# ubc-vision/StableKeypoints

Measured on AMD Instinct MI355X. Metric: images/sec for token-optimization step (SD1.5, 512^2, K=10 kpts), higher is better.
Workload: dtype f32 (fp32 MFMA / VALU throughout; flash attention of the >= 1024-key self-attention layers: 3xbf16 operand split, fp32 accumulate, error <= the fp32 kernel's)

## Files before the change

### include/skp.h

```cpp
#ifndef SKP_H
#define SKP_H

#include <stdint.h>

#ifdef __cplusplus
extern "C" {
#endif

#define SKP_MAX_LAYERS 8
#define SKP_MAX_SUBJECTS 4

#define SKP_E_BADARG (-1)
#define SKP_E_RANGE  (-2)
#define SKP_E_LDS    (-3)

int skp_abi_version(void);

int skp_tune_set(const char* key, int value);
int skp_tune_get(const char* key);

int skp_gemm_nt_f32(const float* A, const float* B, float* C, int M, int N, int K, int Z0, int Z1,
                    int64_t sa0, int64_t sa1, int64_t sam, int64_t sak,
                    int64_t sb0, int64_t sb1, int64_t sbn, int64_t sbk,
                    int64_t sc0, int64_t sc1, int64_t scm, float alpha, void* stream);
// ... 22 lines not shown
int64_t skp_attn_map_bwd_col_workspace(const int* s , int L, int B, int H, int T, int R, int K);
int skp_attn_map_bwd_col_f32(const float* const* S , float* const* dS , const int* s , int L,
                             int B, int H, int T, int R, const int64_t* sel, const float* G, int K, const float* lse,
                             void* workspace, int ldt, void* stream);

int64_t skp_attn_map_bwd_sparse_workspace(const int* s , int L, int B, int H, int T, int R, int K);
int skp_attn_map_bwd_sparse_f32(const float* const* S , float* const* dS , const int* s ,
                                int L, int B, int H, int T, int R, const int64_t* sel, const float* G, int K,
                                const float* lse, void* workspace, int ldt, void* stream);

int skp_unwarp_accumulate_f32(const float* M, const float* theta_inv, int n, int K, int R, int S, float* tot, float* num,
                              int finish, void* stream);

int skp_group_norm_coef_f32(const float* x, const float* off, const float* gamma, const float* beta, float* mean, float* rstd,
                            float* coef, const float* bs, int nblk, int pix, float* workspace, int N, int C, int G, int HW,
                            float eps, void* stream);
int skp_conv3x3_f4_gn_ok(int B, int Cin, int Cout, int H, int W);
int skp_conv3x3_f4_gn_f32(const void* x, const void* U, const void* bias, const void* residual, void* y, float* stats,
                          const float* coef, int B, int Cin, int Cout, int H, int W, void* stream);

int skp_conv3x3_f4r_ok(int B, int Cin, int Cout, int H, int W);
int skp_conv3x3_f4r_filter_f32(const void* w, void* R, int Cout, int Cin, int flip_transpose, void* stream);
int64_t skp_conv3x3_f4r_workspace(int B, int Cin, int Cout, int H, int W);
int skp_conv3x3_f4r_f32(const void* x, const void* R, const void* bias, const void* residual, void* y, void* workspace,
                        int B, int Cin, int Cout, int H, int W, void* stream);

int skp_cross_attn_fwd_f32(const float* q, const float* k, const float* v, float* out, float* lse,
                           int B, int Bk, int H, int N, int T, int d, float scale, void* stream);
int64_t skp_cross_attn_bwd_workspace(int B, int H, int N, int T, int d);
int skp_cross_attn_bwd_f32(const float* q, const float* k, const float* v, const float* out,
                           const float* dout, const float* lse, float* dq, float* dk, float* dv,
                           float* workspace, int B, int Bk, int H, int N, int T, int d, float scale,
                           void* stream);

int skp_attn_map_bwd_ex_f32(const float* const* S , float* const* dS , const int* s ,
                            int L, int B, int H, int T, int R, const float* dM, const float* lse,
                            float* workspace, float* dot_io, int ldt, int64_t m_bstride, int mode, void* stream);

int64_t skp_flash_attn_bwd_workspace(int B, int Bk, int H, int N, int Nk, int d);
int skp_flash_attn_fwd_f32(const float* q, const float* k, const float* v, float* out, float* lse,
                           int B, int Bk, int H, int N, int Nk, int d, float scale, void* stream);
int skp_flash_attn_bwd_f32(const float* q, const float* k, const float* v, const float* out, const float* dout,
                           const float* lse, float* dq, float* dk, float* dv, float* workspace,
                           int B, int Bk, int H, int N, int Nk, int d, float scale, void* stream);
int skp_flash_attn_bwd_ld_f32(const float* q, const float* k, const float* v, const float* out, const float* dout,
                              const float* lse, float* dq, float* dk, float* dv, float* workspace,
                              int B, int Bk, int H, int N, int Nk, int d, float scale, int ldg, void* stream);

int skp_flash_attn_fwd_split_ok(int B, int Bk, int H, int N, int Nk, int d);
int64_t skp_flash_attn_fwd_split_workspace(int B, int Bk, int H, int N, int Nk, int d);
int skp_flash_attn_fwd_split_f32(const float* q, const float* k, const float* v, float* out, float* lse, void* workspace,
                                 int B, int Bk, int H, int N, int Nk, int d, float scale, void* stream);
int skp_flash_attn_bwd_split_ok(int B, int Bk, int H, int N, int Nk, int d);
int64_t skp_flash_attn_bwd_split_workspace(int B, int Bk, int H, int N, int Nk, int d);
int skp_flash_attn_bwd_split_f32(const float* q, const float* k, const float* v, const float* out, const float* dout,
                                 const float* lse, float* dq, float* dk, float* dv, void* workspace, int B, int Bk, int H, int N,
                                 int Nk, int d, float scale, void* stream);
int skp_flash_attn_bwd_split_ld_f32(const float* q, const float* k, const float* v, const float* out, const float* dout,
                                    const float* lse, float* dq, float* dk, float* dv, void* workspace, int B, int Bk, int H,
                                    int N, int Nk, int d, float scale, int ldg, void* stream);

int skp_self_attn_fwd_f32(const float* q, const float* k, const float* v, float* out, float* lse,
                          int B, int H, int N, int d, float scale, void* stream);
int skp_self_attn_bwd_f32(const float* q, const float* k, const float* v, const float* out, const float* dout,
                          const float* lse, float* dq, float* dk, float* dv, float* workspace,
                          int B, int H, int N, int d, float scale, void* stream);
// ... 100 lines not shown
```

### stablekeypoints_amd/_native.py

```python
from __future__ import annotations

import ctypes as C
import os

import torch

_HERE = os.path.dirname(os.path.abspath(__file__))
LIB_PATH = os.environ.get("SKP_LIB_PATH") or os.path.join(_HERE, "csrc", "libskp_hip.so")
ABI_VERSION = 41

_vp, _i, _f, _i64 = C.c_void_p, C.c_int, C.c_float, C.c_int64

SIGNATURES = {
    "skp_abi_version": [],
    "skp_tune_set": [C.c_char_p, _i],
    "skp_tune_get": [C.c_char_p],
    "skp_group_norm_onepass_ok": [_i, _i, _i, _i],
    "skp_gemm_nt_f32": [_vp, _vp, _vp, _i, _i, _i, _i, _i,
                        _i64, _i64, _i64, _i64, _i64, _i64, _i64, _i64, _i64, _i64, _i64, _f, _vp],
    "skp_qk_logits_f32": [_vp, _vp, _vp, _i, _i, _i, _i, _i, _i, _f, _vp],
    "skp_attn_map_fwd_f32": [C.POINTER(_vp), C.POINTER(_i), _i, _i, _i, _i, _i, _vp, _vp, _vp],
    "skp_attn_map_fwd_ex_f32": [C.POINTER(_vp), C.POINTER(_i), _i, _i, _i, _i, _i, _vp, _vp, _vp, _i, _i64, _i, _vp],
    "skp_attn_map_bwd_ex_f32": [C.POINTER(_vp), C.POINTER(_vp), C.POINTER(_i), _i, _i, _i, _i, _i, _vp, _vp, _vp, _vp,
                                _i, _i64, _i, _vp],
    "skp_attn_map_bwd_workspace": [C.POINTER(_i), _i, _i, _i, _i, _i],
    "skp_attn_map_bwd_f32": [C.POINTER(_vp), C.POINTER(_vp), C.POINTER(_i), _i, _i, _i, _i, _i, _vp, _vp, _vp, _vp],
    "skp_group_norm_coef_f32": [_vp, _vp, _vp, _vp, _vp, _vp, _vp, _vp, _i, _i, _vp, _i, _i, _i, _i, _f, _vp],
    "skp_conv3x3_f4_gn_ok": [_i, _i, _i, _i, _i],
    "skp_conv3x3_f4_gn_f32": [_vp, _vp, _vp, _vp, _vp, _vp, _vp, _i, _i, _i, _i, _i, _vp],
    "skp_unwarp_accumulate_f32": [_vp, _vp, _i, _i, _i, _i, _vp, _vp, _i, _vp],
    "skp_attn_map_fwd_wide_f32": [C.POINTER(_vp), C.POINTER(_i), _i, _i, _i, _i, _i, _vp, _vp, _vp, _i, _i, _vp],
    "skp_attn_map_fwd_wide_ok": [C.POINTER(_i), _i, _i, _i],
    "skp_attn_map_bwd_col_ok": [C.POINTER(_i), _i, _i, _i, _i, _i],
    "skp_attn_map_bwd_col_workspace": [C.POINTER(_i), _i, _i, _i, _i, _i, _i],
    "skp_attn_map_bwd_col_f32": [C.POINTER(_vp), C.POINTER(_vp), C.POINTER(_i), _i, _i, _i, _i, _i, _vp, _vp, _i, _vp, _vp,
                                 _i, _vp],
    "skp_attn_map_bwd_sparse_workspace": [C.POINTER(_i), _i, _i, _i, _i, _i, _i],
    "skp_attn_map_bwd_sparse_f32": [C.POINTER(_vp), C.POINTER(_vp), C.POINTER(_i), _i, _i, _i, _i, _i, _vp, _vp, _i, _vp, _vp,
                                    _i, _vp],
    "skp_token_stats_f32": [_vp, _i, _i, _i, _f, _f, _vp, _vp, _vp, _vp],
    "skp_select_tokens": [_vp, _vp, _i, _i, _i, _i, _vp, _vp, _vp],
    "skp_select_tokens_batched": [_vp, _vp, _i, _i, _i, _i, _i, _vp, _vp, _vp],
    "skp_losses_fwd_f32": [_vp, _vp, _vp, _i, _i, _i, _vp, _i, _f, C.POINTER(_f), _vp, _vp, _vp, _vp, _vp],
    "skp_losses_fwd_dev_f32": [_vp, _vp, _vp, _i, _i, _i, _vp, _i, _f, _vp, _vp, _vp, _vp, _vp, _vp],
    "skp_rows_axpy_f32": [_vp, _vp, _i, _i64, _vp, _vp, _vp, _vp, _vp],
    "skp_cross_attn_fwd_f32": [_vp, _vp, _vp, _vp, _vp, _i, _i, _i, _i, _i, _i, _f, _vp],
    "skp_cross_attn_bwd_workspace": [_i, _i, _i, _i, _i],
    "skp_cross_attn_bwd_f32": [_vp, _vp, _vp, _vp, _vp, _vp, _vp, _vp, _vp, _vp, _i, _i, _i, _i, _i, _i, _f, _vp],
    "skp_group_norm_fwd_f32": [_vp, _vp, _vp, _vp, _vp, _vp, _vp, _vp, _i, _i, _i, _i, _f, _i, _vp],
    "skp_group_norm_bwd_f32": [_vp, _vp, _vp, _vp, _vp, _vp, _vp, _vp, _vp, _i, _i, _i, _i, _f, _i, _vp],
    "skp_group_norm_bwd_add_f32": [_vp, _vp, _vp, _vp, _vp, _vp, _vp, _vp, _vp, _vp, _i, _i, _i, _i, _f, _i, _vp],
    "skp_add_bias_residual_f32": [_vp, _vp, _vp, _vp, _i, _i, _i, _vp],
    "skp_add_layer_norm_ok": [_i],
    "skp_add_layer_norm_fwd_f32": [_vp, _vp, _vp, _vp, _vp, _vp, _vp, _i64, _i, _f, _vp],
    "skp_add_layer_norm_bwd_f32": [_vp, _vp, _vp, _vp, _vp, _vp, _i64, _i, _vp],
    "skp_conv3x3_filter_f32": [_vp, _vp, _i, _i, _i, _vp],
    "skp_conv3x3_workspace": [_i, _i, _i, _i, _i, _i],
    "skp_conv3x3_f32": [_vp, _vp, _vp, _vp, _vp, _vp, _i, _i, _i, _i, _i, _i, _vp],
    "skp_conv3x3_f4_filter_f32": [_vp, _vp, _i, _i, _i, _vp],
    "skp_conv3x3_f4_workspace": [_i, _i, _i, _i, _i],
    "skp_conv3x3_f4_f32": [_vp, _vp, _vp, _vp, _vp, _vp, _i, _i, _i, _i, _i, _vp],
    "skp_flash_attn_fwd_split_ok": [_i, _i, _i, _i, _i, _i],
    "skp_flash_attn_fwd_split_workspace": [_i, _i, _i, _i, _i, _i],
    "skp_flash_attn_fwd_split_f32": [_vp, _vp, _vp, _vp, _vp, _vp, _i, _i, _i, _i, _i, _i, C.c_float, _vp],
    "skp_flash_attn_bwd_split_ok": [_i, _i, _i, _i, _i, _i],
    "skp_flash_attn_bwd_split_workspace": [_i, _i, _i, _i, _i, _i],
    "skp_flash_attn_bwd_split_f32": [_vp, _vp, _vp, _vp, _vp, _vp, _vp, _vp, _vp, _vp, _i, _i, _i, _i, _i, _i, _f, _vp],
    "skp_flash_attn_bwd_split_ld_f32": [_vp, _vp, _vp, _vp, _vp, _vp, _vp, _vp, _vp, _vp, _i, _i, _i, _i, _i, _i, _f, _i, _vp],
    "skp_conv3x3_f4r_ok": [_i, _i, _i, _i, _i],
    "skp_conv3x3_f4r_filter_f32": [_vp, _vp, _i, _i, _i, _vp],
    "skp_conv3x3_f4r_workspace": [_i, _i, _i, _i, _i],
    "skp_conv3x3_f4r_f32": [_vp, _vp, _vp, _vp, _vp, _vp, _i, _i, _i, _i, _i, _vp],
    "skp_conv3x3_s2_filter_f32": [_vp, _vp, _i, _i, _vp],
    "skp_conv3x3_s2_f32": [_vp, _vp, _vp, _vp, _i, _i, _i, _i, _i, _i, _vp],
    "skp_conv3x3_s2_workspace": [_i, _i, _i, _i, _i],
    "skp_conv3x3_s2_ws_f32": [_vp, _vp, _vp, _vp, _vp, _i, _i, _i, _i, _i, _i, _vp],
    "skp_conv3x3_s2w_ok": [_i, _i, _i, _i, _i, _i],
    "skp_conv3x3_s2w_filter_f32": [_vp, _vp, _i, _i, _i, _vp],
    "skp_conv3x3_s2w_f32": [_vp, _vp, _vp, _vp, _i, _i, _i, _i, _i, _i, _vp],
    "skp_conv3x3_s2w_stats_f32": [_vp, _vp, _vp, _vp, _vp, _i, _i, _i, _i, _i, _i, _vp],
    "skp_conv3x3_small_f32": [_vp, _vp, _vp, _vp, _i, _i, _i, _i, _i, _vp],
# ... 102 lines not shown
```

### stablekeypoints_amd/csrc/skp_common.h

```cpp
#pragma once
#include <hip/hip_runtime.h>
#include <stdint.h>
#include "../../include/skp.h"

#define SKP_WAVE 64
#define SKP_LOG2E 1.4426950408889634f

typedef float f32x16 __attribute__((ext_vector_type(16)));
typedef float f32x4 __attribute__((ext_vector_type(4)));
typedef float f32x2 __attribute__((ext_vector_type(2)));

enum { SKP_TUNE_WINO_SPLIT = 0, SKP_TUNE_WINO_RAW_MAX_TILES, SKP_TUNE_MAP_BANDS, SKP_TUNE_FA2_TWO_KERNEL_BWD, SKP_TUNE_GN_FOLD_MAX_COUT, SKP_TUNE_CROSS_ATTN_TS,
       SKP_TUNE_CONV_S2W, SKP_TUNE_CONV_UP2, SKP_TUNE_COUNT };
int skp_tune(int key);

static inline int skp_launch_status() {
    hipError_t e = hipGetLastError();
    return e == hipSuccess ? 0 : (int)e;
}

__device__ __forceinline__ void skp_cubic_taps(int dst, float ratio, int n, int idx[4], float w[4]) {
    const float A = -0.75f;
    const float src = ratio * ((float)dst + 0.5f) - 0.5f;
    const float fl = floorf(src);
    const float t = src - fl;
    const int i0 = (int)fl;
    float x = t + 1.0f;
    w[0] = ((A * x - 5.0f * A) * x + 8.0f * A) * x - 4.0f * A;
    x = t;
    w[1] = ((A + 2.0f) * x - (A + 3.0f)) * x * x + 1.0f;
    x = 1.0f - t;
    w[2] = ((A + 2.0f) * x - (A + 3.0f)) * x * x + 1.0f;
    x = 2.0f - t;
    w[3] = ((A * x - 5.0f * A) * x + 8.0f * A) * x - 4.0f * A;
#pragma unroll
    for (int i = 0; i < 4; ++i) {
        int v = i0 - 1 + i;
        idx[i] = v < 0 ? 0 : (v > n - 1 ? n - 1 : v);
    }
}

__device__ __forceinline__ float skp_wave_sum(float v) {
#pragma unroll
    for (int o = 32; o > 0; o >>= 1) v += __shfl_xor(v, o, 64);
    return v;
}
// ... 34 lines not shown
```

### stablekeypoints_amd/csrc/skp_cross_attn.hip

```cpp
#include "skp_attn_tiles.h"

#define SKP_CA_KSPLIT_MAX 16

int skp_gemm_nt_splitk(const float* A, const float* B, float* C, float* partial, int64_t c_elems, int ksplit,
                       int M, int N, int K, int Z0, int Z1,
                       int64_t sa0, int64_t sa1, int64_t sam, int64_t sak,
                       int64_t sb0, int64_t sb1, int64_t sbn, int64_t sbk,
                       int64_t sc0, int64_t sc1, int64_t scm, float alpha, void* stream);

static int ca_ksplit(int N) { int k = N / 256; return k < 1 ? 1 : (k > SKP_CA_KSPLIT_MAX ? SKP_CA_KSPLIT_MAX : k); }

template <int D8, int TT>
__global__ __launch_bounds__(256) void skp_cross_attn_fwd_kernel(const float* __restrict__ q, const float* __restrict__ k,
                                                                 const float* __restrict__ v, float* __restrict__ out,
                                                                 float* __restrict__ lse, int Bk, int H, int N, int T,
                                                                 float scale) {
    using S = CAShape<D8, TT>;
    extern __shared__ __attribute__((aligned(16))) float smem[];
    const int tid = threadIdx.x, wave = tid >> 6, lane = tid & 63, i = lane & 31, hi = lane >> 5;
    const int b = blockIdx.z, h = blockIdx.y, C = H * S::D;
    const int n0 = blockIdx.x * 128 + wave * 32, n = n0 + i;
    const bool nv = n < N;
    const float* qrow = q + ((size_t)b * N + (nv ? n : N - 1)) * C + h * S::D;
    const float sl2 = scale * SKP_LOG2E;
// ... 271 lines not shown
    const float lse2 = lse[((size_t)b * H + h) * N + (nv ? n : N - 1)] * SKP_LOG2E;
#pragma unroll
    for (int r = 0; r < 16; ++r) p[0][r] = (t0 + ca_tok(0, r, hi) < T) ? __builtin_amdgcn_exp2f(p[0][r] - lse2) : 0.f;
    ca_stage_wave<D8>(reg, v + kvoff, t0, T, C, lane);
    {
        f32x4 dov[D8];
#pragma unroll
        for (int j = 0; j < D8; ++j) {
            dov[j] = *(const f32x4*)(dout + rowoff + 8 * j + 4 * hi);
            const f32x4 ov = *(const f32x4*)(out + rowoff + 8 * j + 4 * hi);
            dsum += dov[j][0] * ov[0] + dov[j][1] * ov[1] + dov[j][2] * ov[2] + dov[j][3] * ov[3];
        }
        dsum += __shfl_xor(dsum, 32, 64);
#pragma unroll
        for (int r = 0; r < 16; ++r) dp[0][r] = 0.f;
        ca_swapped_product<D8, 1>(reg, dov, dp, i, hi);
    }
    const size_t stb = ((size_t)b * H + h) * TP * N;
#pragma unroll
    for (int r = 0; r < 16; ++r) {
        dp[0][r] = p[0][r] * (dp[0][r] - dsum);
        if (nv) {
            const size_t o = stb + (size_t)(t0 + ca_tok(0, r, hi)) * N + n;
            Pst[o] = p[0][r];
            dSst[o] = dp[0][r];
        }
    }
    ca_stage_wave<D8>(reg, k + kvoff, t0, T, C, lane);
    f32x16 o[S::CT];
    ca_reg_product<D8, 1>(reg, dp, o, i, hi);
    ca_merge_store<D8, NW>(smem, reg, o, dq, scale, b, h, H, N, n0, wave, lane);
}

static bool ca_use_ts(int B, int H, int N, int T, int d) {
    if (skp_tune(SKP_TUNE_CROSS_ATTN_TS) == 1) return false;
    const int tt = (T + 31) / 32;
    if (tt < 2 || !(d == 80 || d == 160)) return false;
    return (long)((N + 127) / 128) * H * B * 4 < 1024;
}

static int ca_check(int B, int Bk, int H, int N, int T, int d) {
    if (B <= 0 || H <= 0 || N <= 0 || T <= 0 || d <= 0 || (Bk != 1 && Bk != B)) return SKP_E_BADARG;
    if (T > 128 || B > 65535 || H > 65535) return SKP_E_RANGE;
    if (d != 8 && d != 16 && d != 32 && d != 40 && d != 64 && d != 80 && d != 160) return SKP_E_RANGE;
    return 0;
}

#define SKP_CA_DISPATCH(KERNEL, ...)                                                                     \
    {                                                                                                    \
        const int tt = (T + 31) / 32;                                                                    \
        const int tsel = tt <= 1 ? 1 : (tt <= 3 ? 3 : 4);                                                \
        dim3 grid((N + 127) / 128, H, B), block(256);                                                    \
        hipStream_t st = (hipStream_t)stream;                                                            \
        int launched = 0;                                                                                \
        SKP_CA_CASE(KERNEL, 1, 1, __VA_ARGS__) SKP_CA_CASE(KERNEL, 1, 3, __VA_ARGS__) SKP_CA_CASE(KERNEL, 1, 4, __VA_ARGS__)     \
        SKP_CA_CASE(KERNEL, 2, 1, __VA_ARGS__) SKP_CA_CASE(KERNEL, 2, 3, __VA_ARGS__) SKP_CA_CASE(KERNEL, 2, 4, __VA_ARGS__)     \
        SKP_CA_CASE(KERNEL, 4, 1, __VA_ARGS__) SKP_CA_CASE(KERNEL, 4, 3, __VA_ARGS__) SKP_CA_CASE(KERNEL, 4, 4, __VA_ARGS__)     \
        SKP_CA_CASE(KERNEL, 5, 1, __VA_ARGS__) SKP_CA_CASE(KERNEL, 5, 3, __VA_ARGS__) SKP_CA_CASE(KERNEL, 5, 4, __VA_ARGS__)     \
        SKP_CA_CASE(KERNEL, 8, 1, __VA_ARGS__) SKP_CA_CASE(KERNEL, 8, 3, __VA_ARGS__) SKP_CA_CASE(KERNEL, 8, 4, __VA_ARGS__)     \
        SKP_CA_CASE(KERNEL, 10, 1, __VA_ARGS__) SKP_CA_CASE(KERNEL, 10, 3, __VA_ARGS__) SKP_CA_CASE(KERNEL, 10, 4, __VA_ARGS__)  \
        SKP_CA_CASE(KERNEL, 20, 1, __VA_ARGS__) SKP_CA_CASE(KERNEL, 20, 3, __VA_ARGS__) SKP_CA_CASE(KERNEL, 20, 4, __VA_ARGS__)  \
        if (!launched) return SKP_E_RANGE;                                                               \
    }

#define SKP_CA_CASE(KERNEL, D8V, TTV, ...)                                                               \
    if (!launched && d == D8V * 8 && tsel == TTV) {                                                      \
// ... 7 lines not shown
        launched = 1;                                                                                    \
    }

#define SKP_CA_TS_CASE(KERNEL, D8V, NWV, ...)                                                            \
    if (!launched && d == D8V * 8 && nw == NWV) {                                                        \
        const size_t lds = ((size_t)NWV * CATS<D8V>::REG + 2 * NWV * 32) * sizeof(float);                \
        if (lds > 64 * 1024) {                                                                           \
            hipError_t e = hipFuncSetAttribute((const void*)KERNEL<D8V, NWV>,                            \
                                               hipFuncAttributeMaxDynamicSharedMemorySize, (int)lds);    \
            if (e != hipSuccess) return (int)e;                                                          \
        }                                                                                                \
        hipLaunchKernelGGL((KERNEL<D8V, NWV>), dim3((N + 31) / 32, H, B), dim3(64 * NWV), lds, (hipStream_t)stream, __VA_ARGS__); \
        launched = 1;                                                                                    \
    }
#define SKP_CA_TS_DISPATCH(KERNEL, ...)                                                                  \
    {                                                                                                    \
        const int nw = (T + 31) / 32 <= 3 ? ((T + 31) / 32 <= 2 ? 2 : 3) : 4;                            \
        int launched = 0;                                                                                \
        SKP_CA_TS_CASE(KERNEL, 10, 2, __VA_ARGS__) SKP_CA_TS_CASE(KERNEL, 10, 3, __VA_ARGS__) SKP_CA_TS_CASE(KERNEL, 10, 4, __VA_ARGS__) \
        SKP_CA_TS_CASE(KERNEL, 20, 2, __VA_ARGS__) SKP_CA_TS_CASE(KERNEL, 20, 3, __VA_ARGS__) SKP_CA_TS_CASE(KERNEL, 20, 4, __VA_ARGS__) \
        if (!launched) return SKP_E_RANGE;                                                               \
    }

extern "C" int skp_cross_attn_tp(int T) {
    const int tt = (T + 31) / 32;
    return (tt <= 1 ? 1 : (tt <= 3 ? 3 : 4)) * 32;
}

extern "C" int64_t skp_cross_attn_bwd_workspace(int B, int H, int N, int T, int d) {
    if (B <= 0 || H <= 0 || N <= 0 || T <= 0 || T > 128 || d <= 0) return SKP_E_BADARG;
    return (2 * (int64_t)B * H * skp_cross_attn_tp(T) * N + (int64_t)ca_ksplit(N) * B * T * H * d) * (int64_t)sizeof(float);
}

extern "C" int skp_cross_attn_fwd_f32(const float* q, const float* k, const float* v, float* out, float* lse,
                                      int B, int Bk, int H, int N, int T, int d, float scale, void* stream) {
    if (!q || !k || !v || !out || !lse) return SKP_E_BADARG;
    int rc = ca_check(B, Bk, H, N, T, d);
    if (rc) return rc;
    if (ca_use_ts(B, H, N, T, d)) {
        SKP_CA_TS_DISPATCH(skp_cross_attn_fwd_ts_kernel, q, k, v, out, lse, Bk, H, N, T, scale)
        return skp_launch_status();
    }
    SKP_CA_DISPATCH(skp_cross_attn_fwd_kernel, q, k, v, out, lse, Bk, H, N, T, scale)
    return skp_launch_status();
}

extern "C" int skp_cross_attn_bwd_f32(const float* q, const float* k, const float* v, const float* out,
                                      const float* dout, const float* lse, float* dq, float* dk, float* dv,
                                      float* workspace, int B, int Bk, int H, int N, int T, int d, float scale,
                                      void* stream) {
    if (!q || !k || !v || !out || !dout || !lse || !dq || !dk || !dv || !workspace) return SKP_E_BADARG;
    int rc = ca_check(B, Bk, H, N, T, d);
    if (rc) return rc;
    const int TP = skp_cross_attn_tp(T);
    float* Pst = workspace;
    float* dSst = workspace + (size_t)B * H * TP * N;
    if (ca_use_ts(B, H, N, T, d)) {
        SKP_CA_TS_DISPATCH(skp_cross_attn_bwd_ts_kernel, q, k, v, out, dout, lse, dq, Pst, dSst, Bk, H, N, T, TP, scale)
    } else {
        SKP_CA_DISPATCH(skp_cross_attn_bwd_kernel, q, k, v, out, dout, lse, dq, Pst, dSst, Bk, H, N, T, scale)
    }
    rc = skp_launch_status();
    if (rc) return rc;
    const int64_t C = (int64_t)H * d;
    float* part = dSst + (size_t)B * H * TP * N;
    const int ksp = ca_ksplit(N);
// ... 8 lines not shown
```

### stablekeypoints_amd/csrc/skp_select_loss.hip

```cpp
#include "skp_common.h"
#include <string.h>

__device__ __forceinline__ bool skp_better(float v, int i, float bv, int bi) {
    return (v > bv) || (v == bv && i < bi);
}

struct StatsArgs { int T, R, S; float sigma, eps; };

__global__ __launch_bounds__(256) void skp_token_stats_kernel(const float* __restrict__ M, StatsArgs a,
                                                              int32_t* __restrict__ argmax_out,
                                                              float* __restrict__ kl_out, float* __restrict__ ent_out) {
    __shared__ float red_v[4];
    __shared__ int red_i[4];
    __shared__ float red[4];
    __shared__ float s_cy[SKP_MAX_SUBJECTS], s_cx[SKP_MAX_SUBJECTS];
    const int t = blockIdx.x, tid = threadIdx.x, R = a.R, RR = R * R;
    const float* m = M + (size_t)t * RR;
    const float rad = 0.05f * (float)R;
    const float rad2 = rad * rad;
    float maxval0 = 0.f;
    for (int j = 0; j < a.S; ++j) {
        float bv = -INFINITY; int bi = 0x7fffffff;
        for (int p = tid; p < RR; p += 256) {
            const int row = p / R, col = p - row * R;
// ... 338 lines not shown
                                  const int32_t* argmax, int num_subjects, float sigma, const float* theta_inv,
                                  float* partial, float* g_sharp, float* g_eq_a, float* g_eq_b, void* stream) {
    return losses_run(M, Mt, sel, K, T, R, argmax, num_subjects, sigma, theta_inv, nullptr, partial, g_sharp, g_eq_a, g_eq_b, stream);
}

extern "C" int skp_losses_fwd_dev_f32(const float* M, const float* Mt, const int64_t* sel, int K, int T, int R,
                                      const int32_t* argmax, int num_subjects, float sigma, const float* theta_inv_dev,
                                      float* partial, float* g_sharp, float* g_eq_a, float* g_eq_b, void* stream) {
    if (!theta_inv_dev) return SKP_E_BADARG;
    return losses_run(M, Mt, sel, K, T, R, argmax, num_subjects, sigma, nullptr, theta_inv_dev, partial, g_sharp, g_eq_a, g_eq_b, stream);
}

__global__ __launch_bounds__(256) void skp_rows_axpy_kernel(float* __restrict__ dst, const int64_t* __restrict__ sel,
                                                            int64_t n, const float* __restrict__ x,
                                                            const float* __restrict__ a, const float* __restrict__ y,
                                                            const float* __restrict__ b) {
    const int k = blockIdx.y;
    const int64_t i = (int64_t)blockIdx.x * 256 + threadIdx.x;
    if (i >= n) return;
    float v = a[0] * x[(size_t)k * n + i];
    if (y) v += b[0] * y[(size_t)k * n + i];
    dst[(size_t)sel[k] * n + i] += v;
}

extern "C" int skp_rows_axpy_f32(float* dst, const int64_t* sel, int K, int64_t n, const float* x, const float* a,
                                 const float* y, const float* b, void* stream) {
    if (!dst || !sel || !x || !a || K <= 0 || n <= 0 || (y && !b)) return SKP_E_BADARG;
    if (K > 65535) return SKP_E_RANGE;
    hipLaunchKernelGGL(skp_rows_axpy_kernel, dim3((unsigned)((n + 255) / 256), K), dim3(256), 0, (hipStream_t)stream,
                       dst, sel, n, x, a, y, b);
    return skp_launch_status();
}

extern "C" int skp_abi_version(void) { return 41; }

static int g_tune[SKP_TUNE_COUNT] = {0};
static const char* const g_tune_names[SKP_TUNE_COUNT] = {"wino_split", "wino_raw_max_tiles", "map_bands", "fa2_two_kernel_bwd", "gn_fold_max_cout", "cross_attn_ts", "conv_s2w", "conv_up2"};
int skp_tune(int key) { return (key >= 0 && key < SKP_TUNE_COUNT) ? g_tune[key] : 0; }
extern "C" int skp_tune_set(const char* key, int value) {
    if (!key || value < 0) return SKP_E_BADARG;
    for (int i = 0; i < SKP_TUNE_COUNT; ++i)
        if (!strcmp(key, g_tune_names[i])) { g_tune[i] = value; return 0; }
    return SKP_E_RANGE;
}
extern "C" int skp_tune_get(const char* key) {
    if (!key) return SKP_E_BADARG;
    for (int i = 0; i < SKP_TUNE_COUNT; ++i)
        if (!strcmp(key, g_tune_names[i])) return g_tune[i];
    return SKP_E_RANGE;
}
```

### stablekeypoints_amd/ops.py

```python
from __future__ import annotations

import contextlib
import weakref
from typing import List, Sequence, Tuple

import torch

from . import _native as N
from . import routes


def _stream() -> int:
    return torch.cuda.current_stream().cuda_stream


def _dev(t: torch.Tensor, name: str) -> torch.Tensor:
    if not t.is_cuda:
        raise RuntimeError(f"{name}: the StableKeypoints hot path runs on the HIP kernels only "
                           f"(got a {t.device} tensor; there is no CPU fallback)")
    if t.dtype != torch.float32:
        raise RuntimeError(f"{name}: expected float32, got {t.dtype}")
    return t if t.is_contiguous() else t.contiguous()


# ... 491 lines not shown

CROSS_ATTN_HEAD_DIMS = (8, 16, 32, 40, 64, 80, 160)
CROSS_ATTN_MAX_T = 128


def cross_attn_supported(C: int, heads: int, T: int) -> bool:
    return C % heads == 0 and (C // heads) in CROSS_ATTN_HEAD_DIMS


class CrossAttnFn(torch.autograd.Function):

    @staticmethod
    def forward(ctx, q, k, v, heads: int, scale: float):
        q, k, v = _dev(q, "q"), _dev(k, "k"), _dev(v, "v")
        B, Nq, C = q.shape
        Bk, T, _ = k.shape
        out = torch.empty_like(q)
        lse = torch.empty(B, heads, Nq, device=q.device, dtype=torch.float32)
        routes.note("attn.cross", routes.cross_attn_form(B, heads, Nq, T, C // heads, N.lib().skp_tune_get(b"cross_attn_ts") == 1))
        N.check(N.lib().skp_cross_attn_fwd_f32(q.data_ptr(), k.data_ptr(), v.data_ptr(), out.data_ptr(), lse.data_ptr(),
                                               B, Bk, heads, Nq, T, C // heads, float(scale), _stream()),
                "skp_cross_attn_fwd_f32")
        ctx.save_for_backward(q, k, v, out, lse)
        ctx.meta = (heads, float(scale))
        return out

    @staticmethod
    def backward(ctx, dout):
        q, k, v, out, lse = ctx.saved_tensors
        heads, scale = ctx.meta
        dout = _dev(dout, "dout")
        B, Nq, C = q.shape
        Bk, T, _ = k.shape
        dq = torch.empty_like(q)
        dk = torch.empty(B, T, C, device=q.device, dtype=torch.float32)
        dv = torch.empty_like(dk)
        ws = _workspace("skp_cross_attn_bwd_workspace", B, heads, Nq, T, C // heads, device=q.device)
        N.check(N.lib().skp_cross_attn_bwd_f32(q.data_ptr(), k.data_ptr(), v.data_ptr(), out.data_ptr(), dout.data_ptr(),
                                               lse.data_ptr(), dq.data_ptr(), dk.data_ptr(), dv.data_ptr(), _ptr(ws),
                                               B, Bk, heads, Nq, T, C // heads, scale, _stream()),
                "skp_cross_attn_bwd_f32")
        if Bk == 1 and B > 1:
            dk, dv = dk.sum(dim=0, keepdim=True), dv.sum(dim=0, keepdim=True)
        return dq, dk, dv, None, None


def cross_attention(q, k, v, heads: int, scale: float):
    if k.shape[1] > CROSS_ATTN_MAX_T:
        routes.note("attn.cross", "flash")
        return FlashAttnFn.apply(q, k, v, int(heads), float(scale))
    return CrossAttnFn.apply(q, k, v, int(heads), float(scale))


def group_norm_supported(x: torch.Tensor, groups: int) -> bool:
    return (x.is_cuda and x.dtype == torch.float32 and x.dim() == 4 and x.shape[1] % groups == 0
            and (x.shape[2] * x.shape[3]) % 4 == 0 and x.shape[0] * groups <= 65535)


class GroupNormSiLUFn(torch.autograd.Function):

    @staticmethod
    def forward(ctx, x, off, gamma, beta, groups: int, eps: float, silu: bool, blocks=None):
        x = _dev(x, "x")
        Nn, C, Hh, Ww = x.shape
        off_c = _dev(off.reshape(Nn, C), "off") if off is not None else None
        y = torch.empty_like(x)
        mean = torch.empty(Nn, groups, device=x.device, dtype=torch.float32)
        rstd = torch.empty_like(mean)
        routes.note("group_norm", "gn_apply")
        if blocks is not None:
            routes.note("group_norm.stats", "producer_blocks")
            bs, nblk, pix = blocks
            N.check(N.lib().skp_group_norm_fwd_blocks_f32(x.data_ptr(), off_c.data_ptr() if off_c is not None else None,
# ... 889 lines not shown
```

### stablekeypoints_amd/routes.py

```python
from __future__ import annotations

import contextlib
import threading
from typing import Dict, Iterable, Optional, Tuple

KINDS = ("hip", "library", "eager", "host")

_WINO = {"wino4_c128": "hip", "wino4_c64": "hip", "wino4_raw": "hip", "wino2": "hip", "lib": "library"}
_FLASH = {"flash_split": "hip", "flash_f32": "hip", "self_attn_gen1": "hip"}
_BLOCK = {"fused": "hip", "eager": "eager"}

ROUTES: Dict[str, Dict[str, str]] = {
    "conv3x3": dict(_WINO),
    "conv3x3.bwd_data": dict(_WINO),
    "conv_in": {"small": "hip"},
    "conv_out": {"lib": "library", "small_out": "hip"},
    "upsample_conv": {"up2_poly": "hip", "interp_wino": "hip"},
    "conv3x3_s2": {"s2_direct": "hip", "s2_wino": "hip"},
    "conv3x3_s2.bwd_data": {"zero_stuffed": "hip", "lib": "library"},
    "downsample": {"s2_direct": "hip", "eager": "eager"},
    "downsample.untiled": {"eager": "eager"},
    "resnet": dict(_BLOCK),
    "transformer2d": dict(_BLOCK),
    "transformer_block": dict(_BLOCK),
    "time_embedding": {"eager": "eager"},
    "group_norm": {"gn_fold": "hip", "gn_apply": "hip"},
    "group_norm.stats": {"producer_blocks": "hip", "own_pass": "hip"},
    "add_layer_norm": {"add_ln": "hip"},
    "vae.attention": {"lib_core": "library", "eager": "eager"},
    "vae.tail": {"composed": "hip", "eager": "eager"},
    "vae.decoder": dict(_BLOCK),
    "attn.cross": {"ca_token_split": "hip", "ca_plain": "hip", "flash": "hip", "host": "host"},
    "attn.self": {"fused_qkv": "hip", "plain": "hip", "host": "host"},
    "flash.fwd": dict(_FLASH),
    "flash.bwd": dict(_FLASH),
    "map.fwd": {"map_fused": "hip", "map_wide": "hip", "map_groups": "hip", "host": "host"},
    "map.bwd": {"map_dense": "hip", "map_dense_groups": "hip", "map_col": "hip", "map_tok": "hip"},
    "map.select": {"batched": "hip", "per_image": "hip"},
    "map.collect": {"reference_ops": "library", "host": "host"},
    "select.rank": {"select_kernel": "hip", "sort": "library"},
}

DOCUMENTED_LIBRARY_ROUTES: Dict[Tuple[str, str], str] = {
    ("vae.attention", "lib_core"): "VAE mid-block attention, one head of d = 512: baddbmm + softmax + bmm (no flash kernel at that head size)",
    ("conv_out", "lib"): "UNet conv_out 320 -> 4 (full forward only) and a VAE conv_out 512 -> 8 whose tail is not composed: "
                         "output channels below the Winograd kernels' 32-channel blocks",
    ("downsample.untiled", "eager"): "Downsample2D whose input is no multiple of the stride-2 kernel's 16 x 32 pixel tile (SD-1.5 at 512^2: "
                                     "1280 -> 1280 at 16^2 -> 8^2): the module's own stride-2 convolution on MIOpen, forward and backward",
}


class UnexpectedRoute(RuntimeError):

    def __init__(self, found):
        self.found = list(found)
        super().__init__("unexpected kernel routes: " + ", ".join(
            f"{s}/{r} x{n} ({ROUTES[s][r]})" for s, r, n in self.found))


_lock = threading.Lock()
_tables: Dict[int, Dict[str, Dict[str, int]]] = {}
_ident = threading.get_ident
_denied: Optional[frozenset] = None


# ... 128 lines not shown
```

Before: 54.49.

## Add fused single-pass cross-attention backward with per-range dK/dV partials

Adds a fused cross-attention backward kernel that recomputes P from q·K and lse, then computes dP and dS and accumulates dV and dK with MFMA contractions over LDS-transposed tiles, all in one pass per range of query blocks. dQ is written directly. Per-range dK/dV partials go to a workspace and a small sum kernel reduces them, which also folds the Bk==1 batch reduction. The aim is to replace the staged multi-kernel backward and its intermediate materialisation; it costs extra LDS, a partial-sum workspace, and a reduction launch. It is enabled by default for d in {40,64,80} when the token-split path is not selected.

```diff
diff --git a/include/skp.h b/include/skp.h
--- a/include/skp.h
+++ b/include/skp.h
@@ -78,6 +78,13 @@
                            const float* dout, const float* lse, float* dq, float* dk, float* dv,
                            float* workspace, int B, int Bk, int H, int N, int T, int d, float scale,
                            void* stream);
+
+int skp_cross_attn_bwd_fused_ok(int B, int Bk, int H, int N, int T, int d);
+int64_t skp_cross_attn_bwd_fused_workspace(int B, int H, int N, int T, int d, int range_blocks);
+int skp_cross_attn_bwd_fused_f32(const float* q, const float* k, const float* v, const float* out,
+                                 const float* dout, const float* lse, float* dq, float* dk, float* dv,
+                                 float* workspace, int B, int Bk, int H, int N, int T, int d, float scale,
+                                 int range_blocks, void* stream);
 
 int skp_attn_map_bwd_ex_f32(const float* const* S , float* const* dS , const int* s ,
                             int L, int B, int H, int T, int R, const float* dM, const float* lse,
diff --git a/stablekeypoints_amd/_native.py b/stablekeypoints_amd/_native.py
--- a/stablekeypoints_amd/_native.py
+++ b/stablekeypoints_amd/_native.py
@@ -7,7 +7,7 @@
 
 _HERE = os.path.dirname(os.path.abspath(__file__))
 LIB_PATH = os.environ.get("SKP_LIB_PATH") or os.path.join(_HERE, "csrc", "libskp_hip.so")
-ABI_VERSION = 41
+ABI_VERSION = 42
 
 _vp, _i, _f, _i64 = C.c_void_p, C.c_int, C.c_float, C.c_int64
 
@@ -47,6 +47,9 @@
     "skp_cross_attn_fwd_f32": [_vp, _vp, _vp, _vp, _vp, _i, _i, _i, _i, _i, _i, _f, _vp],
     "skp_cross_attn_bwd_workspace": [_i, _i, _i, _i, _i],
     "skp_cross_attn_bwd_f32": [_vp, _vp, _vp, _vp, _vp, _vp, _vp, _vp, _vp, _vp, _i, _i, _i, _i, _i, _i, _f, _vp],
+    "skp_cross_attn_bwd_fused_ok": [_i, _i, _i, _i, _i, _i],
+    "skp_cross_attn_bwd_fused_workspace": [_i, _i, _i, _i, _i, _i],
+    "skp_cross_attn_bwd_fused_f32": [_vp, _vp, _vp, _vp, _vp, _vp, _vp, _vp, _vp, _vp, _i, _i, _i, _i, _i, _i, _f, _i, _vp],
     "skp_group_norm_fwd_f32": [_vp, _vp, _vp, _vp, _vp, _vp, _vp, _vp, _i, _i, _i, _i, _f, _i, _vp],
     "skp_group_norm_bwd_f32": [_vp, _vp, _vp, _vp, _vp, _vp, _vp, _vp, _vp, _i, _i, _i, _i, _f, _i, _vp],
     "skp_group_norm_bwd_add_f32": [_vp, _vp, _vp, _vp, _vp, _vp, _vp, _vp, _vp, _vp, _i, _i, _i, _i, _f, _i, _vp],
diff --git a/stablekeypoints_amd/csrc/skp_common.h b/stablekeypoints_amd/csrc/skp_common.h
--- a/stablekeypoints_amd/csrc/skp_common.h
+++ b/stablekeypoints_amd/csrc/skp_common.h
@@ -11,7 +11,7 @@
 typedef float f32x2 __attribute__((ext_vector_type(2)));
 
 enum { SKP_TUNE_WINO_SPLIT = 0, SKP_TUNE_WINO_RAW_MAX_TILES, SKP_TUNE_MAP_BANDS, SKP_TUNE_FA2_TWO_KERNEL_BWD, SKP_TUNE_GN_FOLD_MAX_COUT, SKP_TUNE_CROSS_ATTN_TS,
-       SKP_TUNE_CONV_S2W, SKP_TUNE_CONV_UP2, SKP_TUNE_COUNT };
+       SKP_TUNE_CONV_S2W, SKP_TUNE_CONV_UP2, SKP_TUNE_CROSS_ATTN_STAGED_BWD, SKP_TUNE_COUNT };
 int skp_tune(int key);
 
 static inline int skp_launch_status() {
diff --git a/stablekeypoints_amd/csrc/skp_cross_attn.hip b/stablekeypoints_amd/csrc/skp_cross_attn.hip
--- a/stablekeypoints_amd/csrc/skp_cross_attn.hip
+++ b/stablekeypoints_amd/csrc/skp_cross_attn.hip
@@ -327,6 +327,188 @@
     ca_merge_store<D8, NW>(smem, reg, o, dq, scale, b, h, H, N, n0, wave, lane);
 }
 
+template <int D8, int TT>
+struct CAFused {
+    using S = CAShape<D8, TT>;
+    static constexpr int LDT = 132;
+    static constexpr int CT16 = (S::D + 15) / 16, NTK = 2 * TT, NTILE = NTK * CT16, NS = (NTILE + 3) / 4;
+    static constexpr int KV = S::TP * S::LDK, TR = S::TP * LDT, XT = CT16 * 16 * LDT;
+    static constexpr bool VRES = (2 * KV + TR + XT) * 4 <= 160 * 1024;
+    static constexpr int VX = KV > XT ? KV : XT;
+    static constexpr int LDS_FLOATS = VRES ? 2 * KV + TR + XT : KV + VX + TR;
+    static_assert(LDS_FLOATS * 4 <= 160 * 1024, "the fused backward's tiles exceed the LDS");
+};
+
+template <int D8, int TT>
+__device__ __forceinline__ void caf_contract(const float* Tr, const float* Xt, f32x4 (&acc)[CAFused<D8, TT>::NS], int wave, int T,
+                                             int lane) {
+    using F = CAFused<D8, TT>;
+    const int l16 = lane & 15, kq = lane >> 4;
+#pragma unroll 1
+    for (int j4 = 0; j4 < 8; ++j4) {
+        f32x4 a[F::NS], x[F::NS];
+#pragma unroll
+        for (int s = 0; s < F::NS; ++s) {
+            const int idx = 4 * s + wave, tk = idx / F::CT16, ct = idx - tk * F::CT16;
+            if (idx < F::NTILE && tk * 16 < T) {
+                a[s] = *(const f32x4*)(Tr + (tk * 16 + l16) * F::LDT + 32 * kq + 4 * j4);
+                x[s] = *(const f32x4*)(Xt + (ct * 16 + l16) * F::LDT + 32 * kq + 4 * j4);
+            }
+        }
+#pragma unroll
+        for (int m = 0; m < 4; ++m)
+#pragma unroll
+            for (int s = 0; s < F::NS; ++s) {
+                const int idx = 4 * s + wave;
+                if (idx < F::NTILE && (idx / F::CT16) * 16 < T)
+                    acc[s] = __builtin_amdgcn_mfma_f32_16x16x4f32(a[s][m], x[s][m], acc[s], 0, 0, 0);
+            }
+    }
+}
+
+template <int D8, int TT>
+__global__ __launch_bounds__(256) void skp_cross_attn_bwd_fused_kernel(const float* __restrict__ q, const float* __restrict__ k,
+                                                                       const float* __restrict__ v, const float* __restrict__ out,
+                                                                       const float* __restrict__ dout, const float* __restrict__ lse,
+                                                                       float* __restrict__ dq, float* __restrict__ part, int Bk, int H,
+                                                                       int N, int T, int RL, float scale) {
+    using S = CAShape<D8, TT>;
+    using F = CAFused<D8, TT>;
+    extern __shared__ __attribute__((aligned(16))) float smem[];
+    float* Ks = smem;
+    float* Vs = smem + F::KV;
+    float* Tr = Vs + (F::VRES ? F::KV : F::VX);
+    float* Xt = F::VRES ? Tr + F::TR : Vs;
+    const int tid = threadIdx.x, wave = __builtin_amdgcn_readfirstlane(tid >> 6), lane = tid & 63, i = lane & 31, hi = lane >> 5;
+    const int b = blockIdx.z, h = blockIdx.y, B = gridDim.z, C = H * S::D;
+    const int NB = (N + 127) / 128, blk0 = blockIdx.x * RL, blk1 = blk0 + RL < NB ? blk0 + RL : NB;
+    const float sl2 = scale * SKP_LOG2E;
+    const size_t kvoff = (Bk == 1 ? 0 : (size_t)b * T * C) + (size_t)h * S::D;
+    ca_stage<D8, TT>(Ks, k + kvoff, T, C, tid);
+    if (F::VRES) ca_stage<D8, TT>(Vs, v + kvoff, T, C, tid);
+    f32x4 accv[F::NS], acck[F::NS];
+#pragma unroll
+    for (int s = 0; s < F::NS; ++s) accv[s] = acck[s] = f32x4{0.f, 0.f, 0.f, 0.f};
+    const int nl = wave * 32 + i;
+    for (int blk = blk0; blk < blk1; ++blk) {
+        const int n0 = blk * 128 + wave * 32, n = n0 + i;
+        const bool nv = n < N;
+        const size_t rowoff = ((size_t)b * N + (nv ? n : N - 1)) * C + h * S::D;
+        f32x16 p[TT], dp[TT];
+        f32x4 qr[D8];
+#pragma unroll
+        for (int j = 0; j < D8; ++j) qr[j] = *(const f32x4*)(q + rowoff + 8 * j + 4 * hi);
+        const float lse2 = lse[((size_t)b * H + h) * N + (nv ? n : N - 1)] * SKP_LOG2E;
+        if (blk == blk0) __syncthreads();
+        {
+            f32x4 qv[D8];
+#pragma unroll
+            for (int j = 0; j < D8; ++j) qv[j] = qr[j] * sl2;
+#pragma unroll
+            for (int tt = 0; tt < TT; ++tt)
+#pragma unroll
+                for (int r = 0; r < 16; ++r) p[tt][r] = 0.f;
+            ca_swapped_product<D8, TT>(Ks, qv, p, i, hi);
+        }
+#pragma unroll
+        for (int tt = 0; tt < TT; ++tt)
+#pragma unroll
+            for (int r = 0; r < 16; ++r)
+                p[tt][r] = (ca_tok(tt, r, hi) < T && nv) ? __builtin_amdgcn_exp2f(p[tt][r] - lse2) : 0.f;
+        f32x4 dov[D8];
+        float dsum = 0.f;
+#pragma unroll
+        for (int j = 0; j < D8; ++j) {
+            dov[j] = *(const f32x4*)(dout + rowoff + 8 * j + 4 * hi);
+            const f32x4 ov = *(const f32x4*)(out + rowoff + 8 * j + 4 * hi);
+            dsum += dov[j][0] * ov[0] + dov[j][1] * ov[1] + dov[j][2] * ov[2] + dov[j][3] * ov[3];
+        }
+        dsum += __shfl_xor(dsum, 32, 64);
+        if (!F::VRES) {
+            __syncthreads();
+            ca_stage<D8, TT>(Vs, v + kvoff, T, C, tid);
+            __syncthreads();
+        }
+#pragma unroll
+        for (int tt = 0; tt < TT; ++tt)
+#pragma unroll
+            for (int r = 0; r < 16; ++r) dp[tt][r] = 0.f;
+        ca_swapped_product<D8, TT>(Vs, dov, dp, i, hi);
+#pragma unroll
+        for (int tt = 0; tt < TT; ++tt)
+#pragma unroll
+            for (int r = 0; r < 16; ++r) dp[tt][r] = p[tt][r] * (dp[tt][r] - dsum);
+        __syncthreads();
+#pragma unroll
+        for (int tt = 0; tt < TT; ++tt)
+#pragma unroll
+            for (int r = 0; r < 16; ++r) Tr[ca_tok(tt, r, hi) * F::LDT + nl] = p[tt][r];
+#pragma unroll
+        for (int j = 0; j < D8; ++j)
+#pragma unroll
+            for (int m = 0; m < 4; ++m) Xt[(8 * j + 4 * hi + m) * F::LDT + nl] = dov[j][m];
+        __syncthreads();
+        caf_contract<D8, TT>(Tr, Xt, accv, wave, T, lane);
+        __syncthreads();
+#pragma unroll
+        for (int tt = 0; tt < TT; ++tt)
+#pragma unroll
+            for (int r = 0; r < 16; ++r) Tr[ca_tok(tt, r, hi) * F::LDT + nl] = dp[tt][r];
+#pragma unroll
+        for (int j = 0; j < D8; ++j)
+#pragma unroll
+            for (int m = 0; m < 4; ++m) Xt[(8 * j + 4 * hi + m) * F::LDT + nl] = qr[j][m];
+        __syncthreads();
+        caf_contract<D8, TT>(Tr, Xt, acck, wave, T, lane);
+        if (dq) {
+            f32x16 o[S::CT];
+            ca_reg_product<D8, TT>(Ks, dp, o, i, hi);
+#pragma unroll
+            for (int ct = 0; ct < S::CT; ++ct) {
+                const int c = ct * 32 + i;
+                if (c < S::D) {
+#pragma unroll
+                    for (int r = 0; r < 16; ++r) {
+                        const int nn = n0 + (r & 3) + 8 * (r >> 2) + 4 * hi;
+                        if (nn < N) dq[((size_t)b * N + nn) * C + h * S::D + c] = scale * o[ct][r];
+                    }
+                }
+            }
+        }
+    }
+    const size_t TD = (size_t)T * S::D, slab = (((size_t)blockIdx.x * B + b) * H + h) * TD, half = (size_t)gridDim.x * B * H * TD;
+    const int l16 = lane & 15, kq = lane >> 4;
+#pragma unroll
+    for (int s = 0; s < F::NS; ++s) {
+        const int idx = 4 * s + wave, tk = idx / F::CT16, ct = idx - tk * F::CT16, c = ct * 16 + l16;
+        if (idx < F::NTILE && c < S::D) {
+#pragma unroll
+            for (int r = 0; r < 4; ++r) {
+                const int t = tk * 16 + 4 * kq + r;
+                if (t < T) {
+                    part[slab + (size_t)t * S::D + c] = accv[s][r];
+                    part[half + slab + (size_t)t * S::D + c] = acck[s][r];
+                }
+            }
+        }
+    }
+}
+
+__global__ __launch_bounds__(256) void skp_cross_attn_bwd_sum_kernel(const float* __restrict__ part, float* __restrict__ dk,
+                                                                     float* __restrict__ dv, int NR, int B, int Bk, int H, int T, int d,
+                                                                     float scale) {
+    const int C = H * d, e = blockIdx.x * 256 + threadIdx.x;
+    if (e >= Bk * T * C) return;
+    const int c = e % d, h = (e / d) % H, t = (e / C) % T, bo = e / (T * C);
+    const size_t TD = (size_t)T * d, half = (size_t)NR * B * H * TD;
+    const float* src = part + (blockIdx.y ? half : 0) + (size_t)h * TD + (size_t)t * d + c;
+    float acc = 0.f;
+    for (int bb = (Bk == 1 ? 0 : bo); bb < (Bk == 1 ? B : bo + 1); ++bb)
+        for (int r = 0; r < NR; ++r) acc += src[((size_t)r * B + bb) * H * TD];
+    if (blockIdx.y) dk[e] = scale * acc;
+    else dv[e] = acc;
+}
+
 static bool ca_use_ts(int B, int H, int N, int T, int d) {
     if (skp_tune(SKP_TUNE_CROSS_ATTN_TS) == 1) return false;
     const int tt = (T + 31) / 32;
@@ -400,6 +582,66 @@
     return (2 * (int64_t)B * H * skp_cross_attn_tp(T) * N + (int64_t)ca_ksplit(N) * B * T * H * d) * (int64_t)sizeof(float);
 }
 
+static bool caf_shape_ok(int B, int Bk, int H, int N, int T, int d) {
+    return ca_check(B, Bk, H, N, T, d) == 0 && (d == 40 || d == 64 || d == 80);
+}
+
+extern "C" int skp_cross_attn_bwd_fused_ok(int B, int Bk, int H, int N, int T, int d) {
+    if (!caf_shape_ok(B, Bk, H, N, T, d)) return 0;
+    if (skp_tune(SKP_TUNE_CROSS_ATTN_STAGED_BWD) == 1) return 0;
+    return ca_use_ts(B, H, N, T, d) ? 0 : 1;
+}
+
+static int caf_range_blocks(int B, int H, int N, int range_blocks) {
+    const int NB = (N + 127) / 128;
+    long rl = range_blocks > 0 ? range_blocks : ((long)NB * H * B + 255) / 256;
+    return (int)(rl < 1 ? 1 : (rl > NB ? NB : rl));
+}
+
+extern "C" int64_t skp_cross_attn_bwd_fused_workspace(int B, int H, int N, int T, int d, int range_blocks) {
+    if (B <= 0 || H <= 0 || N <= 0 || T <= 0 || T > 128 || d <= 0) return SKP_E_BADARG;
+    const int NB = (N + 127) / 128, RL = caf_range_blocks(B, H, N, range_blocks), NR = (NB + RL - 1) / RL;
+    return 2 * (int64_t)NR * B * H * T * d * (int64_t)sizeof(float);
+}
+
+#define SKP_CAF_CASE(D8V, TTV)                                                                           \
+    if (!launched && d == D8V * 8 && tsel == TTV) {                                                      \
+        const size_t lds = CAFused<D8V, TTV>::LDS_FLOATS * sizeof(float);                                \
+        if (lds > 64 * 1024) {                                                                           \
+            hipError_t e = hipFuncSetAttribute((const void*)skp_cross_attn_bwd_fused_kernel<D8V, TTV>,   \
+                                               hipFuncAttributeMaxDynamicSharedMemorySize, (int)lds);    \
+            if (e != hipSuccess) return (int)e;                                                          \
+        }                                                                                                \
+        hipLaunchKernelGGL((skp_cross_attn_bwd_fused_kernel<D8V, TTV>), dim3(NR, H, B), dim3(256), lds, st, q, k, v, out, dout, lse, \
+                           dq, workspace, Bk, H, N, T, RL, scale);                                       \
+        launched = 1;                                                                                    \
+    }
+
+extern "C" int skp_cross_attn_bwd_fused_f32(const float* q, const float* k, const float* v, const float* out,
+                                            const float* dout, const float* lse, float* dq, float* dk, float* dv,
+                                            float* workspace, int B, int Bk, int H, int N, int T, int d, float scale,
+                                            int range_blocks, void* stream) {
+    if (!q || !k || !v || !out || !dout || !lse || !dk || !dv || !workspace) return SKP_E_BADARG;
+    int rc = ca_check(B, Bk, H, N, T, d);
+    if (rc) return rc;
+    if (!caf_shape_ok(B, Bk, H, N, T, d)) return SKP_E_RANGE;
+    const int NB = (N + 127) / 128, RL = caf_range_blocks(B, H, N, range_blocks), NR = (NB + RL - 1) / RL;
+    if (NR > 65535) return SKP_E_RANGE;
+    const int tt = (T + 31) / 32, tsel = tt <= 1 ? 1 : (tt <= 3 ? 3 : 4);
+    hipStream_t st = (hipStream_t)stream;
+    int launched = 0;
+    SKP_CAF_CASE(5, 1) SKP_CAF_CASE(5, 3) SKP_CAF_CASE(5, 4)
+    SKP_CAF_CASE(8, 1) SKP_CAF_CASE(8, 3) SKP_CAF_CASE(8, 4)
+    SKP_CAF_CASE(10, 1) SKP_CAF_CASE(10, 3) SKP_CAF_CASE(10, 4)
+    if (!launched) return SKP_E_RANGE;
+    rc = skp_launch_status();
+    if (rc) return rc;
+    const int elems = Bk * T * H * d;
+    hipLaunchKernelGGL(skp_cross_attn_bwd_sum_kernel, dim3((elems + 255) / 256, 2), dim3(256), 0, st, workspace, dk, dv, NR, B, Bk, H,
+                       T, d, scale);
+    return skp_launch_status();
+}
+
 extern "C" int skp_cross_attn_fwd_f32(const float* q, const float* k, const float* v, float* out, float* lse,
                                       int B, int Bk, int H, int N, int T, int d, float scale, void* stream) {
     if (!q || !k || !v || !out || !lse) return SKP_E_BADARG;
diff --git a/stablekeypoints_amd/csrc/skp_select_loss.hip b/stablekeypoints_amd/csrc/skp_select_loss.hip
--- a/stablekeypoints_amd/csrc/skp_select_loss.hip
+++ b/stablekeypoints_amd/csrc/skp_select_loss.hip
@@ -394,10 +394,10 @@
     return skp_launch_status();
 }
 
-extern "C" int skp_abi_version(void) { return 41; }
+extern "C" int skp_abi_version(void) { return 42; }
 
 static int g_tune[SKP_TUNE_COUNT] = {0};
-static const char* const g_tune_names[SKP_TUNE_COUNT] = {"wino_split", "wino_raw_max_tiles", "map_bands", "fa2_two_kernel_bwd", "gn_fold_max_cout", "cross_attn_ts", "conv_s2w", "conv_up2"};
+static const char* const g_tune_names[SKP_TUNE_COUNT] = {"wino_split", "wino_raw_max_tiles", "map_bands", "fa2_two_kernel_bwd", "gn_fold_max_cout", "cross_attn_ts", "conv_s2w", "conv_up2", "cross_attn_staged_bwd"};
 int skp_tune(int key) { return (key >= 0 && key < SKP_TUNE_COUNT) ? g_tune[key] : 0; }
 extern "C" int skp_tune_set(const char* key, int value) {
     if (!key || value < 0) return SKP_E_BADARG;
diff --git a/stablekeypoints_amd/ops.py b/stablekeypoints_amd/ops.py
--- a/stablekeypoints_amd/ops.py
+++ b/stablekeypoints_amd/ops.py
@@ -547,13 +547,27 @@
         dout = _dev(dout, "dout")
         B, Nq, C = q.shape
         Bk, T, _ = k.shape
+        d = C // heads
+        lib = N.lib()
+        if lib.skp_cross_attn_bwd_fused_ok(B, Bk, heads, Nq, T, d) == 1:
+            routes.note("attn.cross.bwd", "ca_fused")
+            dq = torch.empty_like(q) if ctx.needs_input_grad[0] else None
+            dk = torch.empty(Bk, T, C, device=q.device, dtype=torch.float32)
+            dv = torch.empty_like(dk)
+            ws = _workspace("skp_cross_attn_bwd_fused_workspace", B, heads, Nq, T, d, 0, device=q.device)
+            N.check(lib.skp_cross_attn_bwd_fused_f32(q.data_ptr(), k.data_ptr(), v.data_ptr(), out.data_ptr(), dout.data_ptr(),
+                                                     lse.data_ptr(), _ptr(dq), dk.data_ptr(), dv.data_ptr(), _ptr(ws),
+                                                     B, Bk, heads, Nq, T, d, scale, 0, _stream()),
+                    "skp_cross_attn_bwd_fused_f32")
+            return dq, dk, dv, None, None
+        routes.note("attn.cross.bwd", "ca_staged")
         dq = torch.empty_like(q)
         dk = torch.empty(B, T, C, device=q.device, dtype=torch.float32)
         dv = torch.empty_like(dk)
-        ws = _workspace("skp_cross_attn_bwd_workspace", B, heads, Nq, T, C // heads, device=q.device)
-        N.check(N.lib().skp_cross_attn_bwd_f32(q.data_ptr(), k.data_ptr(), v.data_ptr(), out.data_ptr(), dout.data_ptr(),
-                                               lse.data_ptr(), dq.data_ptr(), dk.data_ptr(), dv.data_ptr(), _ptr(ws),
-                                               B, Bk, heads, Nq, T, C // heads, scale, _stream()),
+        ws = _workspace("skp_cross_attn_bwd_workspace", B, heads, Nq, T, d, device=q.device)
+        N.check(lib.skp_cross_attn_bwd_f32(q.data_ptr(), k.data_ptr(), v.data_ptr(), out.data_ptr(), dout.data_ptr(),
+                                           lse.data_ptr(), dq.data_ptr(), dk.data_ptr(), dv.data_ptr(), _ptr(ws),
+                                           B, Bk, heads, Nq, T, d, scale, _stream()),
                 "skp_cross_attn_bwd_f32")
         if Bk == 1 and B > 1:
             dk, dv = dk.sum(dim=0, keepdim=True), dv.sum(dim=0, keepdim=True)
diff --git a/stablekeypoints_amd/routes.py b/stablekeypoints_amd/routes.py
--- a/stablekeypoints_amd/routes.py
+++ b/stablekeypoints_amd/routes.py
@@ -31,6 +31,7 @@
     "vae.tail": {"composed": "hip", "eager": "eager"},
     "vae.decoder": dict(_BLOCK),
     "attn.cross": {"ca_token_split": "hip", "ca_plain": "hip", "flash": "hip", "host": "host"},
+    "attn.cross.bwd": {"ca_fused": "hip", "ca_staged": "hip"},
     "attn.self": {"fused_qkv": "hip", "plain": "hip", "host": "host"},
     "flash.fwd": dict(_FLASH),
     "flash.bwd": dict(_FLASH),
```

After: 54.76 (median of 4 runs). Within noise of the previous version (+0.5%).
